# facebookresearch/vggsfm

Measured on AMD Instinct MI355X. Metric: BA LM-iterations/sec, higher is better.
Workload: dtype f64

## Files before the change

vggsfm_amd/ba.py:

```python
import copy
import ctypes
from dataclasses import dataclass
from typing import Optional

import math
import os

import numpy as np
import torch

from . import _lib
from .ba_options import LOSS_ID, TERMINATION, BundleAdjustmentOptions

MODEL_ID = {"SIMPLE_PINHOLE": 0, "SIMPLE_RADIAL": 1}
GROUP = 16
CHUNK = 1024
SUB = 32
MIN_CHUNK = 128
OVERLAP_FACTORIZATION = False
OVERLAP_MIN_OBS, OVERLAP_MIN_FRAMES = 1_000_000, 8 * GROUP
TILE_BATCHES = 3
CHOL_CUS = 32


# ... 674 lines not shown
                          CHOL_CUS if (overlap and OVERLAP_FACTORIZATION) else 0)


def _summary_dict(summ, log, n):
    its = [dict(iteration=l.iteration, cost=l.cost, cost_change=l.cost_change, gradient_max_norm=l.gradient_max_norm,
                step_norm=l.step_norm, relative_decrease=l.relative_decrease, radius=l.radius,
                successful=bool(l.successful)) for l in log[:n]]
    return dict(initial_cost=summ.initial_cost, final_cost=summ.final_cost, num_iterations=summ.num_iterations,
                num_successful_steps=summ.num_successful_steps, num_unsuccessful_steps=summ.num_unsuccessful_steps,
                termination=summ.termination, termination_str=TERMINATION.get(summ.termination, "?"),
                n_reduced=summ.n_reduced, iterations=its)


def solve(problem: DeviceProblem, options: Optional[BundleAdjustmentOptions] = None, workspace=None):
    L = _lib.lib()
    options = options or BundleAdjustmentOptions()
    problem.refine_focal = options.refine_focal_length
    problem.refine_extra = options.refine_extra_params
    problem.loss = LOSS_ID[options.loss_function_type]
    problem.loss_scale = options.loss_function_scale
    cp = problem.c_struct()
    co = _c_options(options)
    nbytes = L.vgg_ba_workspace_bytes(ctypes.byref(cp), ctypes.byref(co))
    if workspace is None or workspace.numel() < nbytes:
        workspace = torch.empty(nbytes, dtype=torch.uint8, device=problem.pts.device)
    summ = _lib.BASummary()
    cap = options.solver_options.max_num_iterations + 2
    log = (_lib.BAIteration * cap)()
    _lib.check(L.vgg_ba_solve(ctypes.byref(cp), ctypes.byref(co), workspace, workspace.numel(), ctypes.byref(summ), log, cap,
                              _lib.stream_ptr()), "vgg_ba_solve")
# ... 81 lines not shown
```

vggsfm_amd/csrc/ba.hip:

```cpp
#include <type_traits>

#include "camera_model.hpp"
#include "../../include/vggsfm_amd.h"

namespace vgg {

int cholesky_solve_enqueue(double* A, double* b, int n, double* inv_blocks, int32_t* device_fail, const int32_t* skip_flag,
                           hipStream_t st, const CholOverlap* overlap, int split_a, int split_b, const int32_t* first_blk,
                           bool flags_cleared);
int32_t* cholesky_dataflow_flags(double* ws, int n, size_t* count);
size_t cholesky_workspace_bytes(int n);
void dataflow_signal(int32_t* flag, hipStream_t st);

constexpr int kGroup = 16;
#ifndef VGG_OFFDIAG_OCC
#define VGG_OFFDIAG_OCC 3
#endif
#ifndef VGG_DIAG_OCC
#define VGG_DIAG_OCC 4
#endif
#ifndef VGG_DIAG_FULL_DEPTH
#define VGG_DIAG_FULL_DEPTH 2
#endif
#ifndef VGG_OFF_FULL_DEPTH
// ... 20 lines not shown
#ifndef VGG_CP_OCC
#define VGG_CP_OCC 2
#endif
#ifndef VGG_ABLATE
#define VGG_ABLATE 0
#endif
constexpr int kSub = 32;
constexpr int kMaxWG = 2048;
constexpr int kCamSplitMax = 16;
constexpr int kCamNV = 48;
constexpr int kPackPad = 1024;

struct Ctl {
  double radius, decrease_factor, x_cost, initial_cost, gmax_cams, gmax, cand_cost, mcc, step_norm, rel;
  int32_t iteration, done, termination, need_lin, scale_ready, invalid_streak, num_succ, num_unsucc;
  int32_t linear_fail, accept, rank, world, grad_logged, pad0, pad1, pad2;
};

struct Dims {
  int C, P, O, NI, model, kd, only_k, shared, BDp, n_red, kdsh, loss;
  double loss_scale;
};

constexpr int kYc = 12;
static inline size_t y_slot_doubles(const Dims& d) { return (d.shared || d.kd == 0) ? (size_t)kYc : (size_t)d.BDp * 3; }

struct Ws {
  Ctl* ctl;
  vgg_ba_iteration* log;
  double *cand_q, *cand_t, *cand_intr, *cand_pts;
  double *scale_c, *scale_p, *colsq_c, *dsq_c, *dy;
// ... 35 lines not shown

static Dims make_dims(const vgg_ba_problem* pb) {
  Dims d;
  d.C = pb->num_cams; d.P = pb->num_pts; d.O = pb->num_obs; d.NI = pb->num_intr; d.model = pb->camera_model;
  const int rf = pb->refine_focal ? 1 : 0, rk = (pb->refine_extra && pb->camera_model == kSimpleRadial) ? 1 : 0;
  d.kd = rf + rk;
  d.only_k = (!rf && rk) ? 1 : 0;
  d.shared = (pb->num_intr == 1) ? 1 : 0;
  d.BDp = 6 + d.kd;
  d.n_red = 6 * d.C + d.kd * d.NI;
  d.kdsh = d.shared ? d.kd : 0;
  d.loss = pb->loss; d.loss_scale = pb->loss_scale;
  return d;
}

struct Tuning { int lpp, longt, cam_wgs, point_wgs, tile_rhs; };
static Tuning g_tuning = {0, -1, 0, 0, 2};

static Ws carve(const Dims& d, int max_iters, int num_chunks, int num_segments, void* base) {
  Ws w;
  size_t off = 0;
  auto take = [&](size_t bytes) { size_t o = off; off = align_up(off + bytes, 256); return (char*)base + o; };
  w.ctl = (Ctl*)take(sizeof(Ctl));
  w.log = (vgg_ba_iteration*)take(sizeof(vgg_ba_iteration) * (size_t)(max_iters + 2));
  w.cand_q = (double*)take(8ull * 4 * d.C); w.cand_t = (double*)take(8ull * 3 * d.C);
  w.cand_intr = (double*)take(8ull * 4 * d.NI); w.cand_pts = (double*)take(8ull * 3 * d.P);
  w.scale_c = (double*)take(8ull * d.n_red); w.scale_p = (double*)take(8ull * 3 * d.P);
  w.colsq_c = (double*)take(8ull * d.n_red); w.dsq_c = (double*)take(8ull * d.n_red);
  w.dy = (double*)take(8ull * d.n_red);
  w.active = (uint8_t*)take(d.n_red);
  w.lin_count = (size_t)d.C * d.BDp * d.BDp + (size_t)d.C * d.BDp + d.C;
  w.lin = (double*)take(8ull * w.lin_count);
// ... 284 lines not shown
          R0[1 + m] = -(E[0] * M[0] + E[1] * M[1] + E[2] * M[2]);
          R1[1 + m] = -(E[3] * M[0] + E[4] * M[1] + E[5] * M[2]);
        } else { R0[1 + m] = 0; R1[1 + m] = 0; }
      }
#pragma unroll
      for (int i = 0; i < BD; ++i)
#pragma unroll
        for (int m = 0; m < 1 + KD; ++m) acc[i * (1 + KD) + m] += F[i] * R0[m] + F[BD + i] * R1[m];
    }
  }
  block_sum<NV>(acc, red, tot);
  static_assert(NV <= kCamNV, "cam_split row");
  if (threadIdx.x < NV) w.cam_split[((size_t)c * kCamSplitMax + blockIdx.y) * kCamNV + threadIdx.x] = tot[threadIdx.x];
}

template <int KD, int MODE>
__global__ __launch_bounds__(64) void cam_reduce_kernel(DevProblem pb, Ws w, int split, int point_parts) {
  constexpr int BD = 6 + KD;
  constexpr int NU = BD * (BD + 1) / 2;
  constexpr int NV = (MODE == 0) ? (NU + BD + 1) : (BD * (1 + KD));
  if (w.ctl->done) return;
  if (MODE == 1 && blockIdx.x == 0) {
    double m = 0;
    for (int i = threadIdx.x; i < point_parts; i += 64) m = fmax(m, w.part_B[i]);
    m = wave_max(m);
    if (threadIdx.x == 0) w.gmax_pts[0] = m;
  }
  const Dims& d = pb.d;
  const int c = blockIdx.x, kdsh = d.kdsh;
  if (threadIdx.x >= NV) return;
  double tot = 0.0;
#pragma unroll 8
  for (int sp = 0; sp < split; ++sp) tot += w.cam_split[((size_t)c * kCamSplitMax + sp) * kCamNV + threadIdx.x];
  if (MODE == 0) {
    double* U = w.U + (size_t)c * BD * BD;
    if (threadIdx.x < NU) {
      int i = 0, rem = threadIdx.x;
      while (rem >= BD - i) { rem -= BD - i; ++i; }
      const int k = i + rem;
      U[i * BD + k] = tot;
      U[k * BD + i] = tot;
    } else if (threadIdx.x < NU + BD) {
      w.g[(size_t)c * BD + threadIdx.x - NU] = tot;
    } else {
      w.costc[c] = tot;
    }
  } else {
    const int i = threadIdx.x / (1 + KD), m = threadIdx.x - i * (1 + KD);
    if (m < 1 + kdsh) w.T[((size_t)c * BD + i) * (1 + kdsh) + m] = tot;
  }
}

template <int KD>
__device__ __forceinline__ void prep_body(const DevProblem& pb, const Ws& w, const vgg_ba_options& opt, double* red) {
  constexpr int BD = 6 + KD;
  Ctl* ctl = w.ctl;
  const Dims& d = pb.d;
  const bool first = !ctl->scale_ready;
  double gmax = 0.0, cost = 0.0;
  constexpr int NS = 1 + 2 * (KD > 0 ? KD : 1);
  double sums[NS];
#pragma unroll
  for (int k = 0; k < NS; ++k) sums[k] = 0.0;
  for (int c = threadIdx.x; c < d.C; c += 256) {
// ... 1009 lines not shown
  }
  for (; ch + 1 < c1; ch += 2) { s0 += src[(size_t)ch * R * R]; s1 += src[(size_t)(ch + 1) * R * R]; }
  if (ch < c1) s0 += src[(size_t)ch * R * R];
  const int hi = ri > cj ? ri : cj, lo = ri > cj ? cj : ri;
  double v = -(s0 + s1);
  if constexpr (BD == 6) {
    const double mi = w.active[ri] ? w.scale_c[ri] : 0.0, mj = w.active[cj] ? w.scale_c[cj] : 0.0;
    v *= mi * mj;
  }
  dst[(size_t)hi * n + lo] = v;
}

template <int KD>
__global__ __launch_bounds__(64) void assemble_kernel(DevProblem pb, Ws w, const int32_t* __restrict__ tile_desc, int num_tiles,
                                                      int point_parts) {
  constexpr int BD = 6 + KD;
  __shared__ double rz[6][3];
  __shared__ double rzf[BD];
  if (w.ctl->done) return;
  const int global_terms = (w.ctl->rank == 0);
  const Dims& d = pb.d;
  const int n = d.n_red, kdsh = d.kdsh, tw = 1 + kdsh;
  const int c = blockIdx.x, tid = threadIdx.x;
  const bool trhs = w.tile_rhs != 0;
  if (c < d.C) {
    const double* U = w.U + (size_t)c * BD * BD;
    const double* T = w.T + (size_t)c * BD * tw;
    const int ia = 6 * d.C + (d.shared ? 0 : KD * c);
    const bool full = trhs && !d.shared && KD > 0;
    if (full) {
// ... 17 lines not shown
      if (!trhs) return T[i * tw + m];
      if (!w.active[6 * c + i]) return 0.0;
      return (m == 0 ? (global_terms ? w.g[(size_t)c * BD + i] : 0.0) : 0.0) - rz[i][m];
    };
    for (int e = tid; e < BD * BD; e += 64) {
      const int i = e / BD, j = e - i * BD;
      const int ri = (i < 6) ? 6 * c + i : ia + (i - 6), cj = (j < 6) ? 6 * c + j : ia + (j - 6);
      if (cj > ri) continue;
      if (d.shared && i >= 6 && j >= 6) continue;
      if (trhs && !full && !d.shared && (i >= 6 || j >= 6)) continue;
      double v = 0.0;
      if (global_terms) {
        v = w.scale_c[ri] * w.scale_c[cj] * U[i * BD + j];
        if (ri == cj) v += w.dsq_c[ri];
      }
      if (d.shared && i >= 6) v += w.scale_c[cj] * Tc(j, 1 + (i - 6));
      w.S[(size_t)ri * n + cj] += v;
    }
    if (full) {
      if (tid < BD) {
        const int ri = (tid < 6) ? 6 * c + tid : ia + (tid - 6);
        const double v = (global_terms ? w.scale_c[ri] * w.g[(size_t)c * BD + tid] : 0.0) - rzf[tid];
        w.rhs[ri] += w.active[ri] ? v : 0.0;
      }
    } else {
      if (tid < 6) w.rhs[6 * c + tid] += w.scale_c[6 * c + tid] * Tc(tid, 0);
      if (!trhs && !d.shared && tid >= 6 && tid < BD) w.rhs[ia + tid - 6] += w.scale_c[ia + tid - 6] * T[tid * tw];
    }
  } else {
    if (trhs) {
      double m = 0;
#pragma unroll 8
      for (int i = tid; i < point_parts; i += 64) m = fmax(m, w.part_B[i]);
      m = wave_max(m);
      if (tid == 0) w.gmax_pts[0] = m;
    }
    if (d.shared && KD > 0) {
      const int ia = 6 * d.C;
      constexpr int NS = (KD > 0) ? KD * KD + KD : 1;
      double sums[NS];
#pragma unroll
      for (int i = 0; i < NS; ++i) sums[i] = 0.0;
#pragma unroll 4
      for (int cc = tid; cc < d.C; cc += 64) {
#pragma unroll
        for (int i = 0; i < KD; ++i) {
#pragma unroll
          for (int j = 0; j <= i; ++j) {
            double v = trhs ? 0.0 : w.scale_c[ia + i] * w.T[((size_t)cc * BD + 6 + i) * tw + 1 + j];
            if (global_terms) v += w.scale_c[ia + i] * w.scale_c[ia + j] * w.U[(size_t)cc * BD * BD + (6 + i) * BD + 6 + j];
            sums[i * KD + j] += v;
          }
          sums[KD * KD + i] += trhs ? (global_terms ? w.g[(size_t)cc * BD + 6 + i] : 0.0) : w.T[((size_t)cc * BD + 6 + i) * tw];
        }
      }
      if (trhs) {
#pragma unroll 8
        for (int b = tid; b < point_parts; b += 64) {
          const double* q = w.part_Q + 8 * (size_t)b;
#pragma unroll
          for (int i = 0; i < KD; ++i) {
#pragma unroll
            for (int j = 0; j <= i; ++j) sums[i * KD + j] -= w.scale_c[ia + i] * q[KD + i * KD + j];
            sums[KD * KD + i] -= q[i];
          }
        }
      }
#pragma unroll
      for (int i = 0; i < NS; ++i) sums[i] = wave_sum(sums[i]);
      if (tid == 0) {
#pragma unroll
        for (int i = 0; i < KD; ++i) {
#pragma unroll
          for (int j = 0; j <= i; ++j) {
            double v = sums[i * KD + j];
            if (global_terms && i == j) v += w.dsq_c[ia + i];
            w.S[(size_t)(ia + i) * n + ia + j] += v;
          }
          w.rhs[ia + i] += w.scale_c[ia + i] * sums[KD * KD + i];
        }
      }
    }
  }
}

template <int KD>
__global__ void cam_update_kernel(DevProblem pb, Ws w) {
  if (w.ctl->done) return;
  const Dims& d = pb.d;
  const int c = blockIdx.x * blockDim.x + threadIdx.x;
  if (c > d.C) return;
  double step = 0, xn = 0;
  if (c < d.C) {
    double dl[6];
    for (int k = 0; k < 6; ++k) {
      const int j = 6 * c + k;
      const double dyv = w.active[j] ? w.scale_c[j] * w.rhs[j] : 0.0;
      w.dy[j] = dyv;
// ... 128 lines not shown
      if (G22 != 0.0) {
        const double z2 = ys[2] / G22, z1 = (ys[1] - G12 * z2) / G11, z0 = (ys[0] - G01 * z1 - G02 * z2) / G00;
        s_mcc += 0.5 * (z0 * z0 + z1 * z1 + z2 * z2) + 0.5 * (pd0 * ys[0] * ys[0] + pd1 * ys[1] * ys[1] + pd2 * ys[2] * ys[2]);
      }
    }
  }
  s_mcc = wave_sum(s_mcc); s_step = wave_sum(s_step); s_xn = wave_sum(s_xn);
  if (lane == 0) { red[wave][0] = s_mcc; red[wave][1] = s_step; red[wave][2] = s_xn; }
  __syncthreads();
  if (threadIdx.x < 3) w.part_F[4 * blockIdx.x + 1 + threadIdx.x] = red[0][threadIdx.x] + red[1][threadIdx.x] + red[2][threadIdx.x] + red[3][threadIdx.x];
}

__global__ __launch_bounds__(256) void reduce_step_kernel(Ws w, int nparts, int C) {
  __shared__ double red[4][256];
  if (w.ctl->done) return;
  double s[4] = {0, 0, 0, 0};
  for (int i = threadIdx.x; i < C; i += 256) s[0] += w.cost_cand[i];
  for (int i = threadIdx.x; i < nparts; i += 256)
    for (int k = 1; k < 4; ++k) s[k] += w.part_F[4 * i + k];
  for (int k = 0; k < 4; ++k) red[k][threadIdx.x] = s[k];
  __syncthreads();
  for (int st = 128; st > 0; st >>= 1) {
    if (threadIdx.x < st) for (int k = 0; k < 4; ++k) red[k][threadIdx.x] += red[k][threadIdx.x + st];
    __syncthreads();
  }
  if (threadIdx.x < 4) w.stepsum[threadIdx.x] = red[threadIdx.x][0];
}

__global__ __launch_bounds__(64) void control_kernel(Ws w, vgg_ba_options opt, int C) {
  Ctl* c = w.ctl;
  if (c->done) { if (threadIdx.x == 0) c->accept = 0; return; }
  double step_c = 0, xn_c = 0, mcc_c = 0;
#pragma unroll 4
  for (int i = threadIdx.x; i <= C; i += 64) { step_c += w.cam_part[3 * i]; xn_c += w.cam_part[3 * i + 1]; mcc_c += w.cam_part[3 * i + 2]; }
  step_c = wave_sum(step_c); xn_c = wave_sum(xn_c); mcc_c = wave_sum(mcc_c);
  if (threadIdx.x != 0) return;
  const int it = c->iteration;
  vgg_ba_iteration li;
  li.iteration = it; li.successful = 0; li.cost = c->x_cost; li.cost_change = 0; li.gradient_max_norm = c->gmax;
  li.step_norm = 0; li.relative_decrease = 0; li.radius = c->radius;
  c->accept = 0;
// ... 205 lines not shown
      const int a = (r - P6) / d.kd, g = a / kGroup;
      const int pb0 = GW * g, pb1 = (GW * (g + 1) < P6) ? GW * (g + 1) : P6;
      c += (size_t)pb0 + (size_t)(P6 - pb1) + (size_t)kGroup * d.kd * g;
    }
  }
  return c;
}

static inline int cam_split_for(int C, int O) {
  const int target = g_tuning.cam_wgs > 0 ? g_tuning.cam_wgs : min(1024, max(256, O / 2048));
  const int s = target / (C > 0 ? C : 1);
  return s < 1 ? 1 : (s > kCamSplitMax ? kCamSplitMax : s);
}

template <int KD>
static void launch_linearize(const Launch& L, const DevProblem& dp, const Ws& w) {
  const int split = cam_split_for(L.d.C, L.d.O);
  cam_pass_kernel<KD, 0><<<dim3(L.d.C, split), 256, 0, L.st>>>(dp, w);
  cam_reduce_kernel<KD, 0><<<L.d.C, 64, 0, L.st>>>(dp, w, split, 0);
}

template <int BD>
static void launch_schur_batch(const Launch& L, int batch, hipStream_t st, double* dst, int which = 0) {
  const int32_t* B = L.batches + 6 * batch;
  const int c0 = B[0], cm = B[1], c1 = B[2], t0 = B[3], t1 = B[4];
  if (L.merged_tile_launch && c1 > c0) {
    ProfScope ps(kProfSchurTile, st);
    schur_tile_merged_kernel<BD><<<c1 - c0, 256, 0, st>>>(L.w, L.chunk_desc, L.entries, c0, L.num_segments);
  } else if (cm > c0 && which != 2) {
    ProfScope ps(kProfSchurTile, st);
    schur_tile_kernel<BD, false><<<cm - c0, 256, 0, st>>>(L.w, L.chunk_desc, L.entries, c0, L.num_segments);
  }
  if (!L.merged_tile_launch && c1 > cm && which != 1) {
    ProfScope ps(kProfSchurTileDiag, st);
    schur_tile_kernel<BD, true><<<c1 - cm, 256, 0, st>>>(L.w, L.chunk_desc, L.entries, cm, L.num_segments);
  }
  if (t1 > t0)
    tile_reduce_kernel<BD><<<dim3(div_up(kGroup * BD * kGroup * BD, 256) + (L.w.tile_rhs ? (BD == 6 ? div_up(kGroup * BD * 3, 256) : div_up(2 * kGroup * BD, 256)) : 0),
                                  t1 - t0), 256, 0, st>>>(L.w, L.d.n_red, L.d.C, L.d.kd, L.tile_desc, t0, dst, which == 0 ? -1 : which - 1);
}

template <int KD>
static void launch_schur_batches(const Launch& L, int b0, int b1, hipStream_t st, double* dst, int32_t* done_flags = nullptr,
                                 int which = 0) {
  for (int b = b0; b < b1; ++b) {
    if (L.d.shared || KD == 0) launch_schur_batch<6>(L, b, st, dst, which);
    else launch_schur_batch<6 + KD>(L, b, st, dst, which);
    if (done_flags) dataflow_signal(done_flags + b, st);
  }
}

struct OverlapCtx {
  int chol_cus = 0;
  hipStream_t st_chol = nullptr, st_rest = nullptr;
  hipEvent_t ready = nullptr, chol_done = nullptr;
};
static OverlapCtx* overlap_ctx(const Launch& L) {
  static OverlapCtx ctx[16];
  static bool failed[16] = {};
  const int cus = L.opt.overlap_factorization;
  if (cus <= 0 || cus % 32 != 0 || L.num_batches < 2 || L.num_batches > 8 || L.num_chunks <= 0) return nullptr;
  int dev = 0;
// ... 6 lines not shown
    failed[dev] = true; return nullptr;
  }
  const int words = prop.multiProcessorCount / 32, cw = cus / 32;
  uint32_t mask_chol[16] = {}, mask_rest[16] = {};
  if (words > 16) { failed[dev] = true; return nullptr; }
  for (int i = 0; i < words; ++i) { mask_chol[i] = (i < cw) ? 0xFFFFFFFFu : 0u; mask_rest[i] = (i < cw) ? 0u : 0xFFFFFFFFu; }
  bool ok = hipExtStreamCreateWithCUMask(&c.st_chol, words, mask_chol) == hipSuccess &&
            hipExtStreamCreateWithCUMask(&c.st_rest, words, mask_rest) == hipSuccess &&
            hipEventCreateWithFlags(&c.ready, hipEventDisableTiming) == hipSuccess &&
            hipEventCreateWithFlags(&c.chol_done, hipEventDisableTiming) == hipSuccess;
  if (!ok) { (void)hipGetLastError(); failed[dev] = true; return nullptr; }
  c.chol_cus = cus;
  return &c;
}

template <int KD>
static void phase_schur(const Launch& L, int which = 0) {
  const Dims& d = L.d;
  if (which == 2) {
    if (L.num_chunks > 0) launch_schur_batches<KD>(L, 0, L.num_batches, L.st, L.w.S, nullptr, 2);
    assemble_kernel<KD><<<d.C + 1, 64, 0, L.st>>>(L.dp, L.w, L.tile_desc, L.num_tiles, L.wgB);
    return;
  }
  prep_kernel<KD><<<1, 256, 0, L.st>>>(L.dp, L.w, L.opt);
  {
    ProfScope ps(kProfPointPass, L.st);
    const size_t cam_lds = sizeof(double) * 19 * (size_t)d.C;
    {
      auto launch_cy = [&](auto lpp, auto cy) {
        constexpr int LPP = decltype(lpp)::value;
        constexpr bool CY = decltype(cy)::value;
        const bool longt = long_tracks(LPP, L.d.P, L.d.O);
        const size_t cam_cap = (CY ? 53 : 64) * 1024;
        if (longt && LPP <= 32) {
          if (cam_lds <= cam_cap) point_pass_kernel<KD, true, CY, LPP, (LPP <= 32)><<<L.wgB, 256, cam_lds, L.st>>>(L.dp, L.w, L.opt);
          else point_pass_kernel<KD, false, CY, LPP, (LPP <= 32)><<<L.wgB, 256, 0, L.st>>>(L.dp, L.w, L.opt);
        } else if (cam_lds <= cam_cap) point_pass_kernel<KD, true, CY, LPP><<<L.wgB, 256, cam_lds, L.st>>>(L.dp, L.w, L.opt);
        else point_pass_kernel<KD, false, CY, LPP><<<L.wgB, 256, 0, L.st>>>(L.dp, L.w, L.opt);
      };
      auto launch = [&](auto lpp) {
        if constexpr (KD == 0) launch_cy(lpp, std::true_type{});
        else if (d.shared) launch_cy(lpp, std::true_type{});
        else launch_cy(lpp, std::false_type{});
      };
      if (L.lpp == 8) launch(std::integral_constant<int, 8>{});
      else if (L.lpp == 16) launch(std::integral_constant<int, 16>{});
      else if (L.lpp == 32) launch(std::integral_constant<int, 32>{});
      else launch(std::integral_constant<int, 64>{});
    }
  }
  if (!L.w.tile_rhs) {
    ProfScope ps(kProfCamRhs, L.st);
    const int split = cam_split_for(d.C, d.O);
    cam_pass_kernel<KD, 1><<<dim3(d.C, split), 256, 0, L.st>>>(L.dp, L.w);
    cam_reduce_kernel<KD, 1><<<d.C, 64, 0, L.st>>>(L.dp, L.w, split, L.wgB);
  }
  if (which == 1) {
    if (L.num_chunks > 0) launch_schur_batches<KD>(L, 0, L.num_batches, L.st, L.w.S, nullptr, 1);
    return;
  }
  if (L.num_chunks > 0) {
    if (overlap_ctx(L)) {
      (void)hipMemsetAsync(L.w.S2, 0, sizeof(double) * (size_t)d.n_red * d.n_red, L.st);
      launch_schur_batches<KD>(L, 0, 1, L.st, L.w.S);
    } else {
      launch_schur_batches<KD>(L, 0, L.num_batches, L.st, L.w.S);
    }
  }
  assemble_kernel<KD><<<d.C + 1, 64, 0, L.st>>>(L.dp, L.w, L.tile_desc, L.num_tiles, L.wgB);
}

template <int KD>
static int phase_step(const Launch& L) {
  const Dims& d = L.d;
  size_t chol_flag_count = 0;
  int32_t* chol_flags = cholesky_dataflow_flags(L.w.chol_inv, d.n_red, &chol_flag_count);
  begin_iteration_kernel<<<1, 256, 0, L.st>>>(L.w, L.opt, d.n_red, chol_flags, (int)chol_flag_count);
  int rc;
  if (OverlapCtx* oc = overlap_ctx(L)) {
    (void)hipMemsetAsync(L.w.batch_flags, 0, 64, L.st);
    (void)hipEventRecord(oc->ready, L.st);
    (void)hipStreamWaitEvent(oc->st_rest, oc->ready, 0);
// ... 30 lines not shown
        else point_step_kernel<KD, false, LPP, (LPP <= 32)><<<L.wgB, 256, 0, L.st>>>(L.dp, L.w);
      } else if (cam_lds <= 64 * 1024) point_step_kernel<KD, true, LPP><<<L.wgB, 256, cam_lds, L.st>>>(L.dp, L.w);
      else point_step_kernel<KD, false, LPP><<<L.wgB, 256, 0, L.st>>>(L.dp, L.w);
    };
    if (L.lpp == 8) launch(std::integral_constant<int, 8>{});
    else if (L.lpp == 16) launch(std::integral_constant<int, 16>{});
    else if (L.lpp == 32) launch(std::integral_constant<int, 32>{});
    else launch(std::integral_constant<int, 64>{});
  }
  {
    ProfScope ps(kProfLinearize, L.st);
    DevProblem dc = L.dp;
    dc.cam_q = L.w.cand_q; dc.cam_t = L.w.cand_t; dc.intr = L.w.cand_intr; dc.pts = L.w.cand_pts;
    Ws wc = L.w;
    wc.U = L.w.U_cand; wc.g = L.w.g_cand; wc.costc = L.w.cost_cand;
    launch_linearize<KD>(L, dc, wc);
  }
  reduce_step_kernel<<<1, 256, 0, L.st>>>(L.w, L.wgB, d.C);
  return VGG_OK;
}

static void phase_update(const Launch& L) {
  const Dims& d = L.d;
  control_kernel<<<1, 64, 0, L.st>>>(L.w, L.opt, d.C);
  size_t nmax = (size_t)3 * d.P;
  if ((size_t)4 * d.C > nmax) nmax = (size_t)4 * d.C;
  if ((size_t)4 * d.NI > nmax) nmax = (size_t)4 * d.NI;
  if (L.w.lin_count > nmax) nmax = L.w.lin_count;
  commit_kernel<<<div_up((long)nmax, 256), 256, 0, L.st>>>(L.w, L.cam_q, L.cam_t, L.intr, L.pts, d.C, d.NI, d.P);
}

static int device_cus() {
  static int cus[64] = {0};
// ... 99 lines not shown
    summary->num_log = (h.iteration + 1 < ncopy) ? h.iteration + 1 : ncopy;
  }
  return VGG_OK;
}

}

using namespace vgg;

extern "C" {

int vgg_ba_tuning(int lanes_per_point, int long_tracks, int cam_workgroups, int point_workgroups) {
  if (!(lanes_per_point == 0 || lanes_per_point == 8 || lanes_per_point == 16 || lanes_per_point == 32 || lanes_per_point == 64))
    return VGG_ERR_INVALID_ARGUMENT;
  vgg::g_tuning = vgg::Tuning{lanes_per_point, long_tracks < 0 ? -1 : (long_tracks ? 1 : 0), cam_workgroups > 0 ? cam_workgroups : 0,
                              point_workgroups > 0 ? point_workgroups : 0, vgg::g_tuning.tile_rhs};
  return VGG_OK;
}

int vgg_ba_set_tile_rhs(int enable) {
  vgg::g_tuning.tile_rhs = (enable >= 0 && enable <= 2) ? enable : 1;
  return VGG_OK;
}

int vgg_ba_profile(int enable, int max_launches_per_kernel) {
  for (int k = 0; k < kProfCount; ++k) {
    for (int i = 0; i < g_prof.cap; ++i) { (void)hipEventDestroy(g_prof.start[k][i]); (void)hipEventDestroy(g_prof.stop[k][i]); }
    delete[] g_prof.start[k]; delete[] g_prof.stop[k];
    g_prof.start[k] = g_prof.stop[k] = nullptr; g_prof.n[k] = 0;
  }
  g_prof.cap = 0; g_prof.on = false;
  if (!enable) return VGG_OK;
  if (max_launches_per_kernel <= 0) return VGG_ERR_INVALID_ARGUMENT;
  for (int k = 0; k < kProfCount; ++k) {
    g_prof.start[k] = new hipEvent_t[max_launches_per_kernel];
    g_prof.stop[k] = new hipEvent_t[max_launches_per_kernel];
// ... 33 lines not shown
}

size_t vgg_ba_workspace_bytes(const vgg_ba_problem* problem, const vgg_ba_options* options) {
  if (!problem || !options) return 0;
  const Dims d = make_dims(problem);
  return carve(d, options->max_num_iterations, problem->num_chunks, problem->num_segments, nullptr).total_bytes + 256;
}

int vgg_ba_begin(const vgg_ba_problem* problem, const vgg_ba_options* options, void* workspace, size_t workspace_bytes,
                 int rank, int world_size, void* stream) {
  Launch L;
  int rc = make_launch(problem, options, workspace, (hipStream_t)stream, &L);
  if (rc != VGG_OK) return rc;
  if (workspace_bytes < L.w.total_bytes) return VGG_ERR_WORKSPACE;
  if (world_size < 1 || world_size > kPackPad || rank < 0 || rank >= world_size) return VGG_ERR_INVALID_ARGUMENT;
  VGG_HIP_CHECK(hipMemsetAsync(L.w.Y, 0, L.w.y_bytes, L.st));
  VGG_HIP_CHECK(hipMemsetAsync(L.w.sys, 0, sizeof(double) * L.w.sys_count, L.st));
  init_kernel<<<div_up(L.d.n_red > 0 ? L.d.n_red : 1, 256), 256, 0, L.st>>>(L.dp, L.w, L.opt, rank, world_size);
  (void)dispatch_kd(L.d.kd, [&] { launch_linearize<0>(L, L.dp, L.w); return VGG_OK; },
                    [&] { launch_linearize<1>(L, L.dp, L.w); return VGG_OK; }, [&] { launch_linearize<2>(L, L.dp, L.w); return VGG_OK; });
  VGG_LAUNCH_CHECK();
  return VGG_OK;
}

int vgg_ba_phase(const vgg_ba_problem* problem, const vgg_ba_options* options, void* workspace, int phase, void* stream) {
  Launch L;
  int rc = make_launch(problem, options, workspace, (hipStream_t)stream, &L);
  if (rc != VGG_OK) return rc;
  rc = run_phase(L, phase);
  if (rc != VGG_OK) return rc;
// ... 76 lines not shown
```

Before: 707.5.

## Fuse step-sum reduction into cam reduce and merge tile reduce with assemble

Folds the separate reduce_step kernel into the last-arriving workgroup of cam_reduce_kernel using an atomic ticket, and replaces tile_reduce + prep + assemble with a single tile_assemble_kernel that writes the reduced Schur system, damping and RHS directly when every group has a diagonal tile. The aim is fewer kernel launches and fewer passes over S and rhs per LM iteration. It adds a host-side tile-descriptor check with a sync at begin, per-workspace host state, explicit FMA and contract-off changes that can alter rounding, and a legacy env switch.

```diff
diff --git a/vggsfm_amd/ba.py b/vggsfm_amd/ba.py
--- a/vggsfm_amd/ba.py
+++ b/vggsfm_amd/ba.py
@@ -712,6 +712,9 @@
 
 def solve(problem: DeviceProblem, options: Optional[BundleAdjustmentOptions] = None, workspace=None):
     L = _lib.lib()
+    glue = _hook("VGGSFM_LEGACY_GLUE")
+    if glue is not None:
+        L.vgg_ba_set_tile_rhs(2 | (4 if glue == "1" else 0))
     options = options or BundleAdjustmentOptions()
     problem.refine_focal = options.refine_focal_length
     problem.refine_extra = options.refine_extra_params
diff --git a/vggsfm_amd/csrc/ba.hip b/vggsfm_amd/csrc/ba.hip
--- a/vggsfm_amd/csrc/ba.hip
+++ b/vggsfm_amd/csrc/ba.hip
@@ -1,4 +1,6 @@
+#include <mutex>
 #include <type_traits>
+#include <vector>
 
 #include "camera_model.hpp"
 #include "../../include/vggsfm_amd.h"
@@ -58,7 +60,9 @@
 struct Ctl {
   double radius, decrease_factor, x_cost, initial_cost, gmax_cams, gmax, cand_cost, mcc, step_norm, rel;
   int32_t iteration, done, termination, need_lin, scale_ready, invalid_streak, num_succ, num_unsucc;
-  int32_t linear_fail, accept, rank, world, grad_logged, pad0, pad1, pad2;
+  int32_t linear_fail, accept, rank, world, grad_logged;
+  int32_t step_arrivals;
+  int32_t merged_glue_launches, merged_step_sums;
 };
 
 struct Dims {
@@ -124,8 +128,8 @@
   return d;
 }
 
-struct Tuning { int lpp, longt, cam_wgs, point_wgs, tile_rhs; };
-static Tuning g_tuning = {0, -1, 0, 0, 2};
+struct Tuning { int lpp, longt, cam_wgs, point_wgs, tile_rhs, legacy_glue; };
+static Tuning g_tuning = {0, -1, 0, 0, 2, 0};
 
 static Ws carve(const Dims& d, int max_iters, int num_chunks, int num_segments, void* base) {
   Ws w;
@@ -440,11 +444,30 @@
   if (threadIdx.x < NV) w.cam_split[((size_t)c * kCamSplitMax + blockIdx.y) * kCamNV + threadIdx.x] = tot[threadIdx.x];
 }
 
+template <bool BYPASS>
+__device__ __forceinline__ void reduce_step_body(const Ws& w, int nparts, int C, double (*red)[256]) {
+  auto ld = [](const double* p) -> double {
+    return BYPASS ? __hip_atomic_load(p, __ATOMIC_RELAXED, __HIP_MEMORY_SCOPE_AGENT) : *p;
+  };
+  double s[4] = {0, 0, 0, 0};
+  for (int i = threadIdx.x; i < C; i += 256) s[0] += ld(w.cost_cand + i);
+  for (int i = threadIdx.x; i < nparts; i += 256)
+    for (int k = 1; k < 4; ++k) s[k] += ld(w.part_F + 4 * i + k);
+  for (int k = 0; k < 4; ++k) red[k][threadIdx.x] = s[k];
+  __syncthreads();
+  for (int st = 128; st > 0; st >>= 1) {
+    if (threadIdx.x < st) for (int k = 0; k < 4; ++k) red[k][threadIdx.x] += red[k][threadIdx.x + st];
+    __syncthreads();
+  }
+  if (threadIdx.x < 4) w.stepsum[threadIdx.x] = red[threadIdx.x][0];
+}
+
 template <int KD, int MODE>
-__global__ __launch_bounds__(64) void cam_reduce_kernel(DevProblem pb, Ws w, int split, int point_parts) {
+__global__ __launch_bounds__(MODE == 0 ? 256 : 64) void cam_reduce_kernel(DevProblem pb, Ws w, int split, int point_parts, int step_parts) {
   constexpr int BD = 6 + KD;
   constexpr int NU = BD * (BD + 1) / 2;
   constexpr int NV = (MODE == 0) ? (NU + BD + 1) : (BD * (1 + KD));
+  __shared__ double red[MODE == 0 ? 4 : 1][MODE == 0 ? 256 : 1];
   if (w.ctl->done) return;
   if (MODE == 1 && blockIdx.x == 0) {
     double m = 0;
@@ -454,26 +477,52 @@
   }
   const Dims& d = pb.d;
   const int c = blockIdx.x, kdsh = d.kdsh;
-  if (threadIdx.x >= NV) return;
-  double tot = 0.0;
+  if (threadIdx.x < NV) {
+    double tot = 0.0;
 #pragma unroll 8
-  for (int sp = 0; sp < split; ++sp) tot += w.cam_split[((size_t)c * kCamSplitMax + sp) * kCamNV + threadIdx.x];
-  if (MODE == 0) {
-    double* U = w.U + (size_t)c * BD * BD;
-    if (threadIdx.x < NU) {
-      int i = 0, rem = threadIdx.x;
-      while (rem >= BD - i) { rem -= BD - i; ++i; }
-      const int k = i + rem;
-      U[i * BD + k] = tot;
-      U[k * BD + i] = tot;
-    } else if (threadIdx.x < NU + BD) {
-      w.g[(size_t)c * BD + threadIdx.x - NU] = tot;
+    for (int sp = 0; sp < split; ++sp) tot += w.cam_split[((size_t)c * kCamSplitMax + sp) * kCamNV + threadIdx.x];
+    if (MODE == 0) {
+      double* U = w.U + (size_t)c * BD * BD;
+      if (threadIdx.x < NU) {
+        int i = 0, rem = threadIdx.x;
+        while (rem >= BD - i) { rem -= BD - i; ++i; }
+        const int k = i + rem;
+        U[i * BD + k] = tot;
+        U[k * BD + i] = tot;
+      } else if (threadIdx.x < NU + BD) {
+        w.g[(size_t)c * BD + threadIdx.x - NU] = tot;
+      } else {
+        w.costc[c] = tot;
+      }
     } else {
-      w.costc[c] = tot;
-    }
-  } else {
-    const int i = threadIdx.x / (1 + KD), m = threadIdx.x - i * (1 + KD);
-    if (m < 1 + kdsh) w.T[((size_t)c * BD + i) * (1 + kdsh) + m] = tot;
+      const int i = threadIdx.x / (1 + KD), m = threadIdx.x - i * (1 + KD);
+      if (m < 1 + kdsh) w.T[((size_t)c * BD + i) * (1 + kdsh) + m] = tot;
+    }
+  }
+  if constexpr (MODE == 0) {
+    if (step_parts <= 0) return;
+    asm volatile("s_waitcnt vmcnt(0)" ::: "memory");
+    __syncthreads();
+    if (threadIdx.x == 0) {
+      __builtin_amdgcn_fence(__ATOMIC_RELEASE, "agent");
+      asm volatile("s_waitcnt vmcnt(0)" ::: "memory");
+      const int ticket = __hip_atomic_fetch_add(&w.ctl->step_arrivals, 1, __ATOMIC_ACQ_REL, __HIP_MEMORY_SCOPE_AGENT);
+      const bool last = ticket == (int)gridDim.x - 1;
+      if (last) {
+        __builtin_amdgcn_fence(__ATOMIC_ACQUIRE, "agent");
+        asm volatile("s_waitcnt vmcnt(0)" ::: "memory");
+      }
+      red[0][0] = last ? 1.0 : 0.0;
+    }
+    __syncthreads();
+    const bool last = red[0][0] != 0.0;
+    __syncthreads();
+    if (!last) return;
+    reduce_step_body<true>(w, step_parts, d.C, red);
+    if (threadIdx.x == 0) {
+      w.ctl->merged_step_sums += 1;
+      __hip_atomic_store(&w.ctl->step_arrivals, 0, __ATOMIC_RELAXED, __HIP_MEMORY_SCOPE_AGENT);
+    }
   }
 }
 
@@ -1513,6 +1562,7 @@
 template <int KD>
 __global__ __launch_bounds__(64) void assemble_kernel(DevProblem pb, Ws w, const int32_t* __restrict__ tile_desc, int num_tiles,
                                                       int point_parts) {
+#pragma clang fp contract(off)
   constexpr int BD = 6 + KD;
   __shared__ double rz[6][3];
   __shared__ double rzf[BD];
@@ -1560,7 +1610,7 @@
         v = w.scale_c[ri] * w.scale_c[cj] * U[i * BD + j];
         if (ri == cj) v += w.dsq_c[ri];
       }
-      if (d.shared && i >= 6) v += w.scale_c[cj] * Tc(j, 1 + (i - 6));
+      if (d.shared && i >= 6) v = fma(w.scale_c[cj], Tc(j, 1 + (i - 6)), v);
       w.S[(size_t)ri * n + cj] += v;
     }
     if (full) {
@@ -1570,8 +1620,8 @@
         w.rhs[ri] += w.active[ri] ? v : 0.0;
       }
     } else {
-      if (tid < 6) w.rhs[6 * c + tid] += w.scale_c[6 * c + tid] * Tc(tid, 0);
-      if (!trhs && !d.shared && tid >= 6 && tid < BD) w.rhs[ia + tid - 6] += w.scale_c[ia + tid - 6] * T[tid * tw];
+      if (tid < 6) w.rhs[6 * c + tid] = fma(w.scale_c[6 * c + tid], Tc(tid, 0), w.rhs[6 * c + tid]);
+      if (!trhs && !d.shared && tid >= 6 && tid < BD) w.rhs[ia + tid - 6] = fma(w.scale_c[ia + tid - 6], T[tid * tw], w.rhs[ia + tid - 6]);
     }
   } else {
     if (trhs) {
@@ -1594,7 +1644,7 @@
 #pragma unroll
           for (int j = 0; j <= i; ++j) {
             double v = trhs ? 0.0 : w.scale_c[ia + i] * w.T[((size_t)cc * BD + 6 + i) * tw + 1 + j];
-            if (global_terms) v += w.scale_c[ia + i] * w.scale_c[ia + j] * w.U[(size_t)cc * BD * BD + (6 + i) * BD + 6 + j];
+            if (global_terms) v = fma(w.scale_c[ia + i] * w.scale_c[ia + j], w.U[(size_t)cc * BD * BD + (6 + i) * BD + 6 + j], v);
             sums[i * KD + j] += v;
           }
           sums[KD * KD + i] += trhs ? (global_terms ? w.g[(size_t)cc * BD + 6 + i] : 0.0) : w.T[((size_t)cc * BD + 6 + i) * tw];
@@ -1607,7 +1657,7 @@
 #pragma unroll
           for (int i = 0; i < KD; ++i) {
 #pragma unroll
-            for (int j = 0; j <= i; ++j) sums[i * KD + j] -= w.scale_c[ia + i] * q[KD + i * KD + j];
+            for (int j = 0; j <= i; ++j) sums[i * KD + j] = fma(-w.scale_c[ia + i], q[KD + i * KD + j], sums[i * KD + j]);
             sums[KD * KD + i] -= q[i];
           }
         }
@@ -1623,11 +1673,210 @@
             if (global_terms && i == j) v += w.dsq_c[ia + i];
             w.S[(size_t)(ia + i) * n + ia + j] += v;
           }
-          w.rhs[ia + i] += w.scale_c[ia + i] * sums[KD * KD + i];
+          w.rhs[ia + i] = fma(w.scale_c[ia + i], sums[KD * KD + i], w.rhs[ia + i]);
         }
       }
     }
   }
+}
+
+__device__ __forceinline__ double lm_damping(double colsq, double sc, double radius, const vgg_ba_options& opt) {
+  double dd = colsq * sc * sc;
+  dd = fmin(fmax(dd, opt.min_lm_diagonal), opt.max_lm_diagonal);
+  return dd / radius;
+}
+
+template <int KD, int BD>
+__global__ __launch_bounds__(256) void tile_assemble_kernel(DevProblem pb, Ws w, vgg_ba_options opt,
+                                                            const int32_t* __restrict__ tile_desc, int point_parts) {
+#pragma clang fp contract(off)
+  constexpr int R = kGroup * BD, UBD = 6 + KD;
+  constexpr bool SH = (KD > 0 && BD == 6);
+  constexpr int nb2 = (R * R + 255) / 256;
+  static_assert(BD == 6 || 2 * R <= 256, "the two entry pairs of a full-factor rz row meet in one workgroup");
+  __shared__ double red[256];
+  const Ctl* ctl = w.ctl;
+  if (ctl->done) return;
+  const Dims& d = pb.d;
+  const int C = d.C, n = d.n_red, tid = threadIdx.x;
+  const int global_terms = (ctl->rank == 0);
+  const double radius = ctl->radius;
+  if (blockIdx.y == 0) {
+    if (blockIdx.x == 1) {
+      if (ctl->need_lin && ctl->scale_ready) prep_body<KD>(pb, w, opt, red);
+      return;
+    }
+    if (blockIdx.x != 0) return;
+    double cs[KD > 0 ? KD : 1] = {};
+    if constexpr (SH) {
+      double part[KD];
+#pragma unroll
+      for (int k = 0; k < KD; ++k) part[k] = 0.0;
+      for (int c = tid; c < C; c += 256) {
+#pragma unroll
+        for (int k = 0; k < KD; ++k) part[k] += w.U[(size_t)c * UBD * UBD + (6 + k) * UBD + 6 + k];
+      }
+      const int wv = tid >> 6, ln = tid & 63;
+#pragma unroll
+      for (int k = 0; k < KD; ++k) {
+        const double v = wave_sum(part[k]);
+        if (ln == 0) red[wv * 8 + 1 + k] = v;
+      }
+      __syncthreads();
+#pragma unroll
+      for (int k = 0; k < KD; ++k) cs[k] = (red[1 + k] + red[9 + k]) + (red[17 + k] + red[25 + k]);
+    }
+    if (tid >= 64) return;
+    {
+      double m = 0;
+#pragma unroll 8
+      for (int i = tid; i < point_parts; i += 64) m = fmax(m, w.part_B[i]);
+      m = wave_max(m);
+      if (tid == 0) { w.gmax_pts[0] = m; w.ctl->merged_glue_launches += 1; }
+    }
+    if constexpr (SH) {
+      const int ia = 6 * C;
+      constexpr int NS = KD * KD + KD;
+      double sums[NS];
+#pragma unroll
+      for (int i = 0; i < NS; ++i) sums[i] = 0.0;
+#pragma unroll 4
+      for (int cc = tid; cc < C; cc += 64) {
+#pragma unroll
+        for (int i = 0; i < KD; ++i) {
+#pragma unroll
+          for (int j = 0; j <= i; ++j) {
+            double v = 0.0;
+            if (global_terms) v += w.scale_c[ia + i] * w.scale_c[ia + j] * w.U[(size_t)cc * UBD * UBD + (6 + i) * UBD + 6 + j];
+            sums[i * KD + j] += v;
+          }
+          sums[KD * KD + i] += global_terms ? w.g[(size_t)cc * UBD + 6 + i] : 0.0;
+        }
+      }
+#pragma unroll 8
+      for (int b = tid; b < point_parts; b += 64) {
+        const double* q = w.part_Q + 8 * (size_t)b;
+#pragma unroll
+        for (int i = 0; i < KD; ++i) {
+#pragma unroll
+          for (int j = 0; j <= i; ++j) sums[i * KD + j] = fma(-w.scale_c[ia + i], q[KD + i * KD + j], sums[i * KD + j]);
+          sums[KD * KD + i] -= q[i];
+        }
+      }
+#pragma unroll
+      for (int i = 0; i < NS; ++i) sums[i] = wave_sum(sums[i]);
+      if (tid == 0) {
+#pragma unroll
+        for (int i = 0; i < KD; ++i) {
+          const double dsq = lm_damping(cs[i], w.scale_c[ia + i], radius, opt);
+          w.dsq_c[ia + i] = dsq;
+#pragma unroll
+          for (int j = 0; j <= i; ++j) {
+            double v = sums[i * KD + j];
+            if (global_terms && i == j) v += dsq;
+            w.S[(size_t)(ia + i) * n + ia + j] = 0.0 + v;
+          }
+          w.rhs[ia + i] = fma(w.scale_c[ia + i], sums[KD * KD + i], 0.0);
+        }
+      }
+    }
+    return;
+  }
+  const int tile = blockIdx.y - 1;
+  const int gI = tile_desc[4 * tile], gJ = tile_desc[4 * tile + 1];
+  const int c0 = tile_desc[4 * tile + 2], c1 = tile_desc[4 * tile + 3];
+  if ((int)blockIdx.x >= nb2) {
+    if (gI != gJ) return;
+    constexpr int NE = (BD == 6) ? R * 3 : 2 * R;
+    constexpr size_t STR = (BD == 6) ? (size_t)R * 3 : (size_t)kGroup * 18;
+    const int e = ((int)blockIdx.x - nb2) * 256 + tid;
+    if (BD == 6 && e >= NE) return;
+    const bool live = e < NE;
+    double s0 = 0.0, s1 = 0.0;
+    int ch = c0;
+    const double* src = w.rz_part + (live ? e : 0);
+    for (; ch + 7 < c1; ch += 8) {
+      double v[8];
+#pragma unroll
+      for (int u = 0; u < 8; ++u) v[u] = src[(size_t)(ch + u) * STR];
+#pragma unroll
+      for (int u = 0; u < 8; u += 2) { s0 += v[u]; s1 += v[u + 1]; }
+    }
+    for (; ch + 1 < c1; ch += 2) { s0 += src[(size_t)ch * STR]; s1 += src[(size_t)(ch + 1) * STR]; }
+    if (ch < c1) s0 += src[(size_t)ch * STR];
+    const double rzv = s0 + s1;
+    if (live) w.rz[(size_t)gI * STR + e] = rzv;
+    if constexpr (BD == 6) {
+      const int a = e / 18, i = (e - 18 * a) / 3, col = e - 18 * a - 3 * i;
+      const int c = gI * kGroup + a;
+      if (c >= C) return;
+      const int rj = 6 * c + i;
+      const bool act = w.active[rj] != 0;
+      const double sc = w.scale_c[rj];
+      if (col == 0) {
+        const double Tc = act ? ((global_terms ? w.g[(size_t)c * UBD + i] : 0.0) - rzv) : 0.0;
+        w.rhs[rj] = fma(sc, Tc, 0.0);
+      } else if (SH && col <= KD) {
+        const int k = col - 1, ia = 6 * C;
+        double v = 0.0;
+        if (global_terms) v = w.scale_c[ia + k] * sc * w.U[(size_t)c * UBD * UBD + (6 + k) * UBD + i];
+        const double Tc = act ? (0.0 - rzv) : 0.0;
+        v = fma(sc, Tc, v);
+        w.S[(size_t)(ia + k) * n + rj] = 0.0 + v;
+      }
+    } else {
+      red[tid] = rzv;
+      __syncthreads();
+      if (e >= R) return;
+      const int a = e / BD, t = e - a * BD;
+      const int c = gI * kGroup + a;
+      if (c >= C) return;
+      const double rzf = red[e] + red[e + R];
+      const int ri = (t < 6) ? 6 * c + t : 6 * C + KD * c + (t - 6);
+      const double v = (global_terms ? w.scale_c[ri] * w.g[(size_t)c * UBD + t] : 0.0) - rzf;
+      w.rhs[ri] = 0.0 + (w.active[ri] ? v : 0.0);
+    }
+    return;
+  }
+  const int e = blockIdx.x * 256 + tid;
+  if (e >= R * R) return;
+  const int row = e / R, col = e - row * R;
+  const int a = row / BD, i = row - a * BD, b = col / BD, j = col - b * BD;
+  const int ca = gI * kGroup + a, cb = gJ * kGroup + b;
+  if (ca >= C || cb >= C) return;
+  if (gI == gJ && col > row) return;
+  const int ri = (i < 6) ? 6 * ca + i : 6 * C + KD * ca + (i - 6);
+  const int cj = (j < 6) ? 6 * cb + j : 6 * C + KD * cb + (j - 6);
+  double s0 = 0.0, s1 = 0.0;
+  int ch = c0;
+  const double* src = w.tile_part + e;
+  for (; ch + 7 < c1; ch += 8) {
+    double v[8];
+#pragma unroll
+    for (int u = 0; u < 8; ++u) v[u] = src[(size_t)(ch + u) * R * R];
+#pragma unroll
+    for (int u = 0; u < 8; u += 2) { s0 += v[u]; s1 += v[u + 1]; }
+  }
+  for (; ch + 1 < c1; ch += 2) { s0 += src[(size_t)ch * R * R]; s1 += src[(size_t)(ch + 1) * R * R]; }
+  if (ch < c1) s0 += src[(size_t)ch * R * R];
+  const int hi = ri > cj ? ri : cj, lo = ri > cj ? cj : ri;
+  double v = -(s0 + s1);
+  if constexpr (BD == 6) {
+    const double mi = w.active[ri] ? w.scale_c[ri] : 0.0, mj = w.active[cj] ? w.scale_c[cj] : 0.0;
+    v *= mi * mj;
+  }
+  if (gI == gJ && a == b) {
+    const double* U = w.U + (size_t)ca * UBD * UBD;
+    double t = 0.0;
+    if (global_terms) t = w.scale_c[ri] * w.scale_c[cj] * U[i * UBD + j];
+    if (ri == cj) {
+      const double dsq = lm_damping(U[i * UBD + i], w.scale_c[ri], radius, opt);
+      w.dsq_c[ri] = dsq;
+      if (global_terms) t += dsq;
+    }
+    v = v + t;
+  }
+  w.S[(size_t)hi * n + lo] = v;
 }
 
 template <int KD>
@@ -1786,17 +2035,7 @@
 __global__ __launch_bounds__(256) void reduce_step_kernel(Ws w, int nparts, int C) {
   __shared__ double red[4][256];
   if (w.ctl->done) return;
-  double s[4] = {0, 0, 0, 0};
-  for (int i = threadIdx.x; i < C; i += 256) s[0] += w.cost_cand[i];
-  for (int i = threadIdx.x; i < nparts; i += 256)
-    for (int k = 1; k < 4; ++k) s[k] += w.part_F[4 * i + k];
-  for (int k = 0; k < 4; ++k) red[k][threadIdx.x] = s[k];
-  __syncthreads();
-  for (int st = 128; st > 0; st >>= 1) {
-    if (threadIdx.x < st) for (int k = 0; k < 4; ++k) red[k][threadIdx.x] += red[k][threadIdx.x + st];
-    __syncthreads();
-  }
-  if (threadIdx.x < 4) w.stepsum[threadIdx.x] = red[threadIdx.x][0];
+  reduce_step_body<false>(w, nparts, C, red);
 }
 
 __global__ __launch_bounds__(64) void control_kernel(Ws w, vgg_ba_options opt, int C) {
@@ -2032,14 +2271,14 @@
 }
 
 template <int KD>
-static void launch_linearize(const Launch& L, const DevProblem& dp, const Ws& w) {
+static void launch_linearize(const Launch& L, const DevProblem& dp, const Ws& w, int step_parts = 0) {
   const int split = cam_split_for(L.d.C, L.d.O);
   cam_pass_kernel<KD, 0><<<dim3(L.d.C, split), 256, 0, L.st>>>(dp, w);
-  cam_reduce_kernel<KD, 0><<<L.d.C, 64, 0, L.st>>>(dp, w, split, 0);
+  cam_reduce_kernel<KD, 0><<<L.d.C, 256, 0, L.st>>>(dp, w, split, 0, step_parts);
 }
 
 template <int BD>
-static void launch_schur_batch(const Launch& L, int batch, hipStream_t st, double* dst, int which = 0) {
+static void launch_schur_batch(const Launch& L, int batch, hipStream_t st, double* dst, int which = 0, bool sums = true) {
   const int32_t* B = L.batches + 6 * batch;
   const int c0 = B[0], cm = B[1], c1 = B[2], t0 = B[3], t1 = B[4];
   if (L.merged_tile_launch && c1 > c0) {
@@ -2053,17 +2292,17 @@
     ProfScope ps(kProfSchurTileDiag, st);
     schur_tile_kernel<BD, true><<<c1 - cm, 256, 0, st>>>(L.w, L.chunk_desc, L.entries, cm, L.num_segments);
   }
-  if (t1 > t0)
+  if (t1 > t0 && sums)
     tile_reduce_kernel<BD><<<dim3(div_up(kGroup * BD * kGroup * BD, 256) + (L.w.tile_rhs ? (BD == 6 ? div_up(kGroup * BD * 3, 256) : div_up(2 * kGroup * BD, 256)) : 0),
                                   t1 - t0), 256, 0, st>>>(L.w, L.d.n_red, L.d.C, L.d.kd, L.tile_desc, t0, dst, which == 0 ? -1 : which - 1);
 }
 
 template <int KD>
 static void launch_schur_batches(const Launch& L, int b0, int b1, hipStream_t st, double* dst, int32_t* done_flags = nullptr,
-                                 int which = 0) {
+                                 int which = 0, bool sums = true) {
   for (int b = b0; b < b1; ++b) {
-    if (L.d.shared || KD == 0) launch_schur_batch<6>(L, b, st, dst, which);
-    else launch_schur_batch<6 + KD>(L, b, st, dst, which);
+    if (L.d.shared || KD == 0) launch_schur_batch<6>(L, b, st, dst, which, sums);
+    else launch_schur_batch<6 + KD>(L, b, st, dst, which, sums);
     if (done_flags) dataflow_signal(done_flags + b, st);
   }
 }
@@ -2100,6 +2339,45 @@
   return &c;
 }
 
+struct HostSolve { const void* ws; bool prep_pending, all_diag; };
+constexpr int kHostSolves = 64;
+static HostSolve g_host_solves[kHostSolves];
+static int g_host_solve_next = 0;
+static std::mutex g_host_solve_mutex;
+
+static void host_solve_begin(const void* ws, bool all_diag) {
+  std::lock_guard<std::mutex> lock(g_host_solve_mutex);
+  HostSolve* h = nullptr;
+  for (HostSolve& e : g_host_solves) if (e.ws == ws) h = &e;
+  if (!h) { h = &g_host_solves[g_host_solve_next]; g_host_solve_next = (g_host_solve_next + 1) % kHostSolves; }
+  *h = HostSolve{ws, true, all_diag};
+}
+static bool host_solve_state(const void* ws, bool* prep_pending, bool* all_diag) {
+  std::lock_guard<std::mutex> lock(g_host_solve_mutex);
+  for (HostSolve& e : g_host_solves) {
+    if (e.ws != ws || !ws) continue;
+    *prep_pending = e.prep_pending; *all_diag = e.all_diag;
+    e.prep_pending = false;
+    return true;
+  }
+  return false;
+}
+
+static bool every_group_has_diagonal_tile(const Launch& L) {
+  const int G = div_up(L.d.C, kGroup);
+  if (!L.tile_desc || L.num_tiles < G) return false;
+  std::vector<int32_t> td((size_t)4 * L.num_tiles);
+  if (hipMemcpyAsync(td.data(), L.tile_desc, sizeof(int32_t) * td.size(), hipMemcpyDeviceToHost, L.st) != hipSuccess ||
+      hipStreamSynchronize(L.st) != hipSuccess) { (void)hipGetLastError(); return false; }
+  std::vector<char> seen((size_t)G, 0);
+  for (int t = 0; t < L.num_tiles; ++t) {
+    const int gI = td[4 * t], gJ = td[4 * t + 1];
+    if (gI == gJ && gI >= 0 && gI < G && td[4 * t + 3] > td[4 * t + 2]) seen[gI] = 1;
+  }
+  for (char c : seen) if (!c) return false;
+  return true;
+}
+
 template <int KD>
 static void phase_schur(const Launch& L, int which = 0) {
   const Dims& d = L.d;
@@ -2108,7 +2386,11 @@
     assemble_kernel<KD><<<d.C + 1, 64, 0, L.st>>>(L.dp, L.w, L.tile_desc, L.num_tiles, L.wgB);
     return;
   }
-  prep_kernel<KD><<<1, 256, 0, L.st>>>(L.dp, L.w, L.opt);
+  bool prep_pending = true, all_diag = false;
+  const bool known = host_solve_state(L.w.ctl, &prep_pending, &all_diag);
+  const bool fused = which == 0 && known && all_diag && !g_tuning.legacy_glue && L.w.tile_rhs && L.num_chunks > 0 &&
+                     L.num_batches == 1 && L.batches[3] == 0 && L.batches[4] == L.num_tiles;
+  if (!fused || prep_pending) prep_kernel<KD><<<1, 256, 0, L.st>>>(L.dp, L.w, L.opt);
   {
     ProfScope ps(kProfPointPass, L.st);
     const size_t cam_lds = sizeof(double) * 19 * (size_t)d.C;
@@ -2139,7 +2421,7 @@
     ProfScope ps(kProfCamRhs, L.st);
     const int split = cam_split_for(d.C, d.O);
     cam_pass_kernel<KD, 1><<<dim3(d.C, split), 256, 0, L.st>>>(L.dp, L.w);
-    cam_reduce_kernel<KD, 1><<<d.C, 64, 0, L.st>>>(L.dp, L.w, split, L.wgB);
+    cam_reduce_kernel<KD, 1><<<d.C, 64, 0, L.st>>>(L.dp, L.w, split, L.wgB, 0);
   }
   if (which == 1) {
     if (L.num_chunks > 0) launch_schur_batches<KD>(L, 0, L.num_batches, L.st, L.w.S, nullptr, 1);
@@ -2150,8 +2432,19 @@
       (void)hipMemsetAsync(L.w.S2, 0, sizeof(double) * (size_t)d.n_red * d.n_red, L.st);
       launch_schur_batches<KD>(L, 0, 1, L.st, L.w.S);
     } else {
-      launch_schur_batches<KD>(L, 0, L.num_batches, L.st, L.w.S);
-    }
+      launch_schur_batches<KD>(L, 0, L.num_batches, L.st, L.w.S, nullptr, 0, !fused);
+    }
+  }
+  if (fused) {
+    auto launch = [&](auto bd) {
+      constexpr int BD = decltype(bd)::value;
+      constexpr int R = kGroup * BD;
+      const int gx = div_up(R * R, 256) + (BD == 6 ? div_up(R * 3, 256) : div_up(2 * R, 256));
+      tile_assemble_kernel<KD, BD><<<dim3(gx, 1 + L.num_tiles), 256, 0, L.st>>>(L.dp, L.w, L.opt, L.tile_desc, L.wgB);
+    };
+    if (d.shared || KD == 0) launch(std::integral_constant<int, 6>{});
+    else launch(std::integral_constant<int, 6 + KD>{});
+    return;
   }
   assemble_kernel<KD><<<d.C + 1, 64, 0, L.st>>>(L.dp, L.w, L.tile_desc, L.num_tiles, L.wgB);
 }
@@ -2212,9 +2505,9 @@
     dc.cam_q = L.w.cand_q; dc.cam_t = L.w.cand_t; dc.intr = L.w.cand_intr; dc.pts = L.w.cand_pts;
     Ws wc = L.w;
     wc.U = L.w.U_cand; wc.g = L.w.g_cand; wc.costc = L.w.cost_cand;
-    launch_linearize<KD>(L, dc, wc);
-  }
-  reduce_step_kernel<<<1, 256, 0, L.st>>>(L.w, L.wgB, d.C);
+    launch_linearize<KD>(L, dc, wc, g_tuning.legacy_glue ? 0 : L.wgB);
+  }
+  if (g_tuning.legacy_glue) reduce_step_kernel<<<1, 256, 0, L.st>>>(L.w, L.wgB, d.C);
   return VGG_OK;
 }
 
@@ -2344,12 +2637,14 @@
   if (!(lanes_per_point == 0 || lanes_per_point == 8 || lanes_per_point == 16 || lanes_per_point == 32 || lanes_per_point == 64))
     return VGG_ERR_INVALID_ARGUMENT;
   vgg::g_tuning = vgg::Tuning{lanes_per_point, long_tracks < 0 ? -1 : (long_tracks ? 1 : 0), cam_workgroups > 0 ? cam_workgroups : 0,
-                              point_workgroups > 0 ? point_workgroups : 0, vgg::g_tuning.tile_rhs};
+                              point_workgroups > 0 ? point_workgroups : 0, vgg::g_tuning.tile_rhs, vgg::g_tuning.legacy_glue};
   return VGG_OK;
 }
 
 int vgg_ba_set_tile_rhs(int enable) {
-  vgg::g_tuning.tile_rhs = (enable >= 0 && enable <= 2) ? enable : 1;
+  const bool known = enable >= 0 && enable <= 7 && (enable & 3) <= 2;
+  vgg::g_tuning.tile_rhs = known ? (enable & 3) : 1;
+  vgg::g_tuning.legacy_glue = (known && (enable & 4)) ? 1 : 0;
   return VGG_OK;
 }
 
@@ -2413,6 +2708,7 @@
   if (rc != VGG_OK) return rc;
   if (workspace_bytes < L.w.total_bytes) return VGG_ERR_WORKSPACE;
   if (world_size < 1 || world_size > kPackPad || rank < 0 || rank >= world_size) return VGG_ERR_INVALID_ARGUMENT;
+  host_solve_begin(L.w.ctl, L.w.tile_rhs && !g_tuning.legacy_glue && every_group_has_diagonal_tile(L));
   VGG_HIP_CHECK(hipMemsetAsync(L.w.Y, 0, L.w.y_bytes, L.st));
   VGG_HIP_CHECK(hipMemsetAsync(L.w.sys, 0, sizeof(double) * L.w.sys_count, L.st));
   init_kernel<<<div_up(L.d.n_red > 0 ? L.d.n_red : 1, 256), 256, 0, L.st>>>(L.dp, L.w, L.opt, rank, world_size);
```

Result: faster. 716.0 (median of 6 runs) (+1.2%).
